# FoundationVision/OmniTokenizer

Measured on AMD Instinct MI355X. Metric: patches/sec encode+decode, higher is better.
Workload: dtype f32 (fp32 operands as 2 fp16 planes, 3 fp16-MFMA products, fp32 accumulate; spatial attention likewise; VQ: fp16-MFMA screen + exact fp32 re-evaluation, ids bit-exact); 1 GPU; C3: B=32/GPU 17x256x256 clips, stage-2 (imagenet_k600 arch: ttww/tttt, pt=4, rope, n_codes=8192), encode + decode; 32 distinct clips per rank; global_batch=32, parallelism=clip-sharded x1

## Files before the change

### omnitokenizer_amd/csrc/common.cpp

```cpp
#include "common.h"
#include "../../include/omnitok_debug.h"
#include <limits.h>
#include <string.h>

namespace omnitok {
static thread_local char g_err[1024] = "";

void set_error(const char *fmt, ...) {
    va_list ap;
    va_start(ap, fmt);
    vsnprintf(g_err, sizeof(g_err), fmt, ap);
    va_end(ap);
}
}

#include <map>
#include <mutex>
#include <utility>

namespace omnitok {
static std::mutex g_attr_mu;
static std::map<std::pair<const void *, int>, int> g_attr_bytes;
static std::map<int, int> g_dev_cus;

int set_max_dynamic_lds(const void *kernel, int bytes) {
    int dev = 0;
    OT_HIP(hipGetDevice(&dev));
    std::lock_guard<std::mutex> lk(g_attr_mu);
    int &have = g_attr_bytes[std::make_pair(kernel, dev)];
    if (bytes > have) {
        OT_HIP(hipFuncSetAttribute(kernel, hipFuncAttributeMaxDynamicSharedMemorySize, bytes));
        have = bytes;
    }
    return OMNITOK_OK;
}

int current_device_cus(int *n_cu) {
    int dev = 0;
    OT_HIP(hipGetDevice(&dev));
    std::lock_guard<std::mutex> lk(g_attr_mu);
    auto it = g_dev_cus.find(dev);
    if (it == g_dev_cus.end()) {
        int n = 0;
        OT_HIP(hipDeviceGetAttribute(&n, hipDeviceAttributeMultiprocessorCount, dev));
        it = g_dev_cus.emplace(dev, n).first;
    }
    *n_cu = it->second;
    return OMNITOK_OK;
}
}

#define OT_OPTIONS(X)                   \
    X(gemm_variant, false, INT_MIN)     \
    X(gemm_lds_pad_kb, false, INT_MIN)  \
    X(gemm_gn, false, INT_MIN)          \
    X(gemm_small, false, INT_MIN)       \
    X(vq_split, false, INT_MIN)         \
    X(vq_variant, false, INT_MIN)       \
    X(vq_screen, false, INT_MIN)        \
    X(vq_screen_split, false, INT_MIN)  \
    X(x3_tile, false, INT_MIN)          \
    X(h2_tile, false, INT_MIN)          \
    X(peg_variant, false, INT_MIN)      \
    X(gemm_mode, true, INT_MIN)         \
    X(attn_mode, true, INT_MIN)         \
    X(attn_h2_variant, false, INT_MIN)  \
    X(attn_vpack, false, INT_MIN)       \
    X(attn_window_mode, false, INT_MIN) \
    X(gemm_pl, true, INT_MIN)           \
    X(qkv_pl, false, INT_MIN)           \
    X(pl_min_tokens, true, INT_MIN)     \
    X(pl_cfg, true, INT_MIN)            \
    X(pl_tail, true, INT_MIN)           \
    X(pl_stagger, false, INT_MIN)       \
    X(sp_small_blocks, true, INT_MIN)   \
    X(temporal_chunk, true, INT_MIN)    \
    X(temporal_fused, false, INT_MIN)   \
    X(temporal_kernel, false, INT_MIN)  \
    X(prevq_fuse, true, INT_MIN)        \
    X(lm_wide_u, true, INT_MIN)         \
    X(lm_balance, true, INT_MIN)        \
    X(lm_ksliced, true, INT_MIN)        \
    X(lm_mfma, true, INT_MIN)           \
    X(lm_mfma_mult, true, INT_MIN)      \
    X(lm_ks_deep, true, INT_MIN)        \
    X(lm_attn_short, true, INT_MIN)     \
    X(lm_attn_waves, true, INT_MIN)     \
    X(lm_loss_chunk_rows, true, 1)

namespace omnitok {
extern long long *g_gemm_trace;
void lm_trace_reset();
#define OT_OPTION_DECL(name, readable, min) extern int g_##name;
OT_OPTIONS(OT_OPTION_DECL)
#undef OT_OPTION_DECL

struct Option {
    const char *name;
    int *value;
    bool readable;
    int min;
};
#define OT_OPTION_ROW(name, readable, min) {#name, &g_##name, readable, min},
static const Option g_options[] = {OT_OPTIONS(OT_OPTION_ROW)};
#undef OT_OPTION_ROW

static const Option *find_option(const char *name) {
    for (const Option &o : g_options)
        if (!strcmp(name, o.name)) return &o;
    return nullptr;
}
}

extern "C" int omnitok_set_option(const char *name, int value) {
    if (!name) return OMNITOK_ERR_INVALID;
    const omnitok::Option *o = omnitok::find_option(name);
    if (!o) {
        omnitok::set_error("set_option: unknown option %s", name);
        return OMNITOK_ERR_INVALID;
    }
    OT_CHECK_ARG(value >= o->min, "set_option: %s %d, expected at least %d", name, value, o->min);
    *o->value = value;
    return OMNITOK_OK;
}

extern "C" int omnitok_get_option(const char *name, int *value) {
    if (!name || !value) return OMNITOK_ERR_INVALID;
    const omnitok::Option *o = omnitok::find_option(name);
    if (!o || !o->readable) {
// ... 16 lines not shown
```

### omnitokenizer_amd/csrc/engine.h

```cpp
#pragma once
#include "common.h"

#include <map>
#include <string>
#include <vector>
#include <algorithm>
#include <cmath>
#include <cstring>
#include <cstdlib>
#include <iterator>

namespace omnitok {

struct DevTensor {
    void *p = nullptr;
    std::vector<int64_t> shape;
    bool is_int64 = false;
    int64_t numel() const {
        int64_t n = 1;
        for (auto s : shape) n *= s;
        return n;
    }
};

// ... 20 lines not shown
    const float *ng, *nb, *wqkv, *wproj, *bproj, *bias_dense;
    const float *wqkv_fold = nullptr, *fold_b = nullptr, *fold_u = nullptr;
    float ln_bound = 0.0f, ao_bound = 0.0f;
    float q_bound = 0.0f, k_bound = 0.0f;
};
struct LayerFF {
    const float *lw, *lb, *w1p, *w2p;
    float ln_bound = 0.0f, h_bound = 0.0f;
};
struct H2W {
    const void *pl = nullptr;
    const float *sc = nullptr;
};
struct ABound {
    float stat = 0.0f;
    const float *dev = nullptr;
    int64_t rpc = 0;
};
struct Layer {
    char kind;
    LayerT t;
    LayerW w;
    LayerFF ff;
    const float *pool_w = nullptr, *pool_b = nullptr;
};

struct Geo {
    bool defer_t, defer_s;
    int p_enc, pt_enc, p_dec, pt_dec, n_pool;
};
struct TransformerW {
    std::vector<Layer> layers;
    const float *og, *ob;
    float out_bound = 0.0f;
};

struct TimingRec {
    std::string name;
    hipEvent_t a, b;
    double work;
};

}

using namespace omnitok;

struct omnitok_engine {
    omnitok_config cfg;
    std::map<std::string, std::vector<int64_t>> spec;
    std::map<std::string, DevTensor> w;
    std::vector<void *> owned;
    std::vector<void *> retired;
    int opt_gemm_mode = -1, opt_attn_mode = -1, opt_attn_vpack = -1, opt_gemm_pl = -1;
    int opt_pl_min_tokens = -1, opt_temporal_chunk = -1;
    bool finalized = false;
    int inner_pad = 0;
    TransformerW enc_s, enc_t, dec_s, dec_t;
    const float *pe_w[2] = {nullptr, nullptr}, *pe_b[2] = {nullptr, nullptr};
    int pe_k[2] = {0, 0}, pe_ld[2] = {0, 0};
    const float *px_w[2] = {nullptr, nullptr}, *px_b[2] = {nullptr, nullptr};
    float *cb_packed = nullptr, *cb_ee = nullptr, *cb_screen = nullptr, *alibi = nullptr;
    float *dq_table = nullptr;
    std::map<int, std::pair<float *, float *>> rope;
    std::map<std::string, float *> bias_tables;
    Buf X, X2, Y, QKV, AO, HD, Z, ST;
    float *ext_ws = nullptr;
    int64_t ext_ws_bytes = 0;
    std::map<const float *, H2W> h2w;
    std::map<const float *, H2W> plw;
    float pe_bound[2] = {0.0f, 0.0f};
    float *bounds = nullptr;
    int bound_next = 0, bound_clips = 0, bound_cap = 0;
    float *range_scratch = nullptr;
    int *err_flag = nullptr;
    bool timing = false;
    std::vector<TimingRec> recs;
    std::vector<hipEvent_t> pool;
};

namespace omnitok {

constexpr int N_BOUND_LAUNCHES = 64;

extern int g_gemm_mode, g_attn_mode, g_attn_vpack, g_gemm_pl, g_pl_min_tokens, g_temporal_chunk, g_prevq_fuse, g_vq_screen, g_temporal_fused;
extern int g_qkv_pl, g_attn_window_mode;

constexpr int64_t PL_BLOCK_BYTES = 8192;
inline int64_t pl_row_offset(int64_t row0, int K) { return (row0 / 64) * (int64_t)(K / 32) * PL_BLOCK_BYTES; }
inline int64_t pad256(int64_t rows) { return (rows + 255) / 256 * 256; }

Geo geometry(const omnitok_config &c);
bool walk_enc_grid(const char *block, int *gh, int *gw, int64_t *peak);
void add_transformer_spec(omnitok_engine *e, const std::string &prefix, const std::string &block, bool rel);
bool key_unused(const omnitok_engine *e, const std::string &k);
int alloc_f(omnitok_engine *e, float **out, int64_t n);
int ensure(Buf &b, int64_t n);
const char *k_embed(const omnitok_config &c);
const char *k_pre_w(const omnitok_config &c);
const char *k_pre_b(const omnitok_config &c);
const char *k_post_w(const omnitok_config &c);
const char *k_post_b(const omnitok_config &c);
const float *W(omnitok_engine *e, const std::string &k);
int build_transformer(omnitok_engine *e, TransformerW &tw, const std::string &prefix, const std::string &block, bool spatial,
                      hipStream_t stream);
int build_patch_operands(omnitok_engine *e, hipStream_t stream);
int get_rope(omnitok_engine *e, int N, const float **cosp, const float **sinp, hipStream_t stream);
int get_bias_table(omnitok_engine *e, const std::string &prefix, int gh, int gw, const float **out, hipStream_t stream);
int gemm_mode_of(const omnitok_engine *e);
int attn_mode_of(const omnitok_engine *e);
int attn_vpack_of(const omnitok_engine *e);
int gemm_pl_of(const omnitok_engine *e, int64_t tokens);
bool x3_ok(const omnitok_engine *e, int N, int K, int flags);
float *next_bounds(omnitok_engine *e);
struct VPack {
    void *planes; int col0, n_tokens, heads; float bound; const float *bound_dev;
};
struct EgGemm {
    const float *a = nullptr, *w = nullptr, *bias = nullptr, *residual = nullptr;
    int64_t lda = 0, ldw = 0, ldr = 0;
    float *c = nullptr;
    int64_t ldc = 0;
    int64_t M = 0;
    int N = 0, K = 0, flags = 0;
    int64_t rpg = 0, gstride = 0, goff = 0;
    ABound ab;
    const float *ln_stats = nullptr, *ln_g = nullptr, *ln_b = nullptr;
    int ln_cols = 0;
    float ln_bound = 0.0f;
    float *c2 = nullptr;
    int64_t ldc2 = 0;
    int split_col = 0;
    const VPack *vpk = nullptr;
};
int eg_gemm(omnitok_engine *e, const EgGemm &g, hipStream_t stream, bool *vpacked = nullptr);
struct PreVqFuse {
    const float *w, *b;
    float *z;
// ... 45 lines not shown
```

### omnitokenizer_amd/csrc/engine.hip

```cpp
#include "engine.h"

namespace omnitok {

int reset_bounds(omnitok_engine *e, int B, hipStream_t stream) {
    if (B > e->bound_cap) {
        if (e->bounds) e->retired.push_back(e->bounds);
        e->bounds = nullptr;
        const int cap = B > 1024 ? B : 1024;
        OT_HIP(hipMalloc(reinterpret_cast<void **>(&e->bounds), (size_t)2 * cap * N_BOUND_LAUNCHES * sizeof(float)));
        e->bound_cap = cap;
    }
    e->bound_clips = B;
    e->bound_next = 0;
    if (int rc = device_fill_u32(e->bounds, 0u, (int64_t)2 * B * N_BOUND_LAUNCHES, stream)) return rc;
    return OMNITOK_OK;
}

void workspace_widths(const omnitok_engine *e, int64_t (&wd)[8]) {
    const omnitok_config &c = e->cfg;
    const int D = c.dim;
    const Geo g = geometry(c);
    const int kenc = ((c.image_channels * g.p_enc * g.p_enc * g.pt_enc + 31) / 32) * 32;
    const int kdec = c.image_channels * g.p_dec * g.p_dec * g.pt_dec;
    const int kmax = kenc > kdec ? kenc : kdec;
// ... 403 lines not shown
extern "C" int64_t omnitok_engine_workspace_need_encode(omnitok_engine *e, int B, int F, int H, int W_) {
    if (!e) return -1;
    const int64_t L = encode_peak_tokens(e, B, F, H, W_);
    return L < 0 ? -1 : workspace_bytes_for(e, L);
}

extern "C" int64_t omnitok_engine_workspace_need_decode(omnitok_engine *e, int B, int T, int gh, int gw) {
    if (!e || T < 1 || gh < 1 || gw < 1) return -1;
    const Geo g = geometry(e->cfg);
    const int T2 = g.defer_t ? 1 + (T - 1) * 2 : T, up = g.defer_s ? 2 : 1;
    return workspace_bytes_for(e, (int64_t)B * T2 * gh * up * gw * up);
}

extern "C" int omnitok_engine_set_workspace(omnitok_engine *e, void *dev_ptr, int64_t bytes) {
    OT_CHECK_ARG(e, "set_workspace: null engine");
    OT_CHECK_ARG((dev_ptr == nullptr) == (bytes == 0) && bytes >= 0, "set_workspace: pointer / size mismatch");
    OT_CHECK_ARG((reinterpret_cast<uintptr_t>(dev_ptr) & 255) == 0, "set_workspace: the block must be 256-byte aligned");
    Buf *bufs[8] = {&e->X, &e->X2, &e->Y, &e->QKV, &e->AO, &e->HD, &e->Z, &e->ST};
    if (!e->ext_ws)
        for (Buf *b : bufs)
            if (b->p) (void)hipFree(b->p);
    for (Buf *b : bufs) {
        b->p = nullptr;
        b->cap = 0;
    }
    e->ext_ws = static_cast<float *>(dev_ptr);
    e->ext_ws_bytes = bytes;
    return OMNITOK_OK;
}

extern "C" int64_t omnitok_engine_workspace_bytes(omnitok_engine *e) {
    int64_t n = 0;
    for (Buf *b : {&e->X, &e->X2, &e->Y, &e->QKV, &e->AO, &e->HD, &e->Z, &e->ST}) n += b->cap * 4;
    return n;
}

extern "C" int omnitok_engine_set_option(omnitok_engine *e, const char *name, int value) {
    OT_CHECK_ARG(e && name, "engine_set_option: null pointer");
    OT_CHECK_ARG(value >= -1, "engine_set_option: value %d (-1 = follow the process default)", value);
    const std::string n(name);
    if (n == "gemm_mode") {
        OT_CHECK_ARG(value <= 2, "engine_set_option: gemm_mode %d", value);
        e->opt_gemm_mode = value;
    } else if (n == "attn_mode") {
        e->opt_attn_mode = value;
    } else if (n == "attn_vpack") {
        e->opt_attn_vpack = value;
    } else if (n == "gemm_pl") {
        e->opt_gemm_pl = value;
    } else if (n == "pl_min_tokens") {
        e->opt_pl_min_tokens = value;
    } else if (n == "temporal_chunk") {
        e->opt_temporal_chunk = value;
    } else {
        set_error("engine_set_option: %s is not a per-engine option (gemm_mode, attn_mode, attn_vpack, gemm_pl, pl_min_tokens, "
                  "temporal_chunk)", name);
        return OMNITOK_ERR_INVALID;
    }
    return OMNITOK_OK;
}

extern "C" int omnitok_engine_set_timing(omnitok_engine *e, int enabled) {
    OT_CHECK_ARG(e, "set_timing: null engine");
    e->timing = enabled != 0;
    return OMNITOK_OK;
}

extern "C" int omnitok_engine_check_ids(omnitok_engine *e, omnitok_stream_t stream_) {
    hipStream_t stream = static_cast<hipStream_t>(stream_);
    int flag = 0;
    OT_HIP(hipMemcpyAsync(&flag, e->err_flag, sizeof(int), hipMemcpyDeviceToHost, stream));
    OT_HIP(hipStreamSynchronize(stream));
    if (flag) {
        if (int rc = device_fill_u32(e->err_flag, 0u, 1, stream)) return rc;
        set_error("decode: token id out of range [0, %d)", e->cfg.n_codes);
        return OMNITOK_ERR_INVALID;
    }
    return OMNITOK_OK;
}

extern "C" int omnitok_engine_timing_report(omnitok_engine *e, char *buf, int buflen) {
    OT_CHECK_ARG(e && buf && buflen > 0, "timing_report: bad arguments");
    OT_HIP(hipDeviceSynchronize());
    struct Acc { int calls = 0; double ms = 0, work = 0; };
    std::map<std::string, Acc> acc;
    for (auto &r : e->recs) {
        float ms = 0;
        (void)hipEventElapsedTime(&ms, r.a, r.b);
        Acc &a = acc[r.name];
        a.calls++;
        a.ms += ms;
        a.work += r.work;
        e->pool.push_back(r.a);
        e->pool.push_back(r.b);
    }
    e->recs.clear();
    std::string s;
    char line[256];
    for (auto &kv : acc) {
        snprintf(line, sizeof(line), "%s %d %.6f %.6e\n", kv.first.c_str(), kv.second.calls, kv.second.ms,
                 kv.second.work);
        s += line;
    }
    strncpy(buf, s.c_str(), buflen - 1);
    buf[buflen - 1] = 0;
    return OMNITOK_OK;
}
```

### omnitokenizer_amd/csrc/engine_run.hip

```cpp
#include "engine.h"

namespace omnitok {

int g_gemm_mode = 2;
int g_attn_mode = 1;
int g_attn_vpack = 1;
int g_gemm_pl = 1;
int g_pl_min_tokens = 0;
int g_temporal_chunk = 0;
int g_prevq_fuse = 1;
int g_temporal_fused = 1;
int g_qkv_pl = 1;
int g_attn_window_mode = 1;

int gemm_mode_of(const omnitok_engine *e) { return e->opt_gemm_mode >= 0 ? e->opt_gemm_mode : g_gemm_mode; }
int attn_mode_of(const omnitok_engine *e) { return e->opt_attn_mode >= 0 ? e->opt_attn_mode : g_attn_mode; }
int attn_vpack_of(const omnitok_engine *e) { return e->opt_attn_vpack >= 0 ? e->opt_attn_vpack : g_attn_vpack; }
int gemm_pl_of(const omnitok_engine *e, int64_t tokens) {
    const int min_tokens = e->opt_pl_min_tokens >= 0 ? e->opt_pl_min_tokens : g_pl_min_tokens;
    return (e->opt_gemm_pl >= 0 ? e->opt_gemm_pl : g_gemm_pl) && tokens >= min_tokens;
}
static int temporal_chunk_of(const omnitok_engine *e) { return e->opt_temporal_chunk >= 0 ? e->opt_temporal_chunk : g_temporal_chunk; }

bool x3_ok(const omnitok_engine *e, int N, int K, int flags) {
    return gemm_mode_of(e) >= 1 && N % 32 == 0 && K % 32 == 0 && !(flags & OMNITOK_GEMM_LEAKY) &&
           (!(flags & OMNITOK_GEMM_GEGLU) || N % 64 == 0);
}

float *next_bounds(omnitok_engine *e) {
    if (e->bound_next >= N_BOUND_LAUNCHES) return nullptr;
    return e->bounds + (int64_t)2 * e->bound_clips * (e->bound_next++);
}

int eg_gemm(omnitok_engine *e, const EgGemm &g, hipStream_t stream, bool *vpacked) {
    omnitok_row_gemm d = {};
    d.a = g.a; d.lda = g.lda; d.w = g.w; d.ldw = g.ldw;
    d.bias = g.bias; d.residual = g.residual; d.ldr = g.ldr; d.c = g.c; d.ldc = g.ldc;
    d.M = g.M; d.N = g.N; d.K = g.K; d.flags = g.flags;
    d.a_rows_per_group = g.rpg; d.a_group_stride = g.gstride; d.a_group_offset = g.goff;
    d.a_bound = g.ab.stat; d.a_bound_dev = g.ab.dev; d.a_bound_stride = 2; d.a_rows_per_clip = g.ab.rpc;
    d.ln_stats = g.ln_stats; d.ln_gamma = g.ln_g; d.ln_beta = g.ln_b; d.ln_cols = g.ln_cols; d.ln_bound = g.ln_bound;
    d.c2 = g.c2; d.ldc2 = g.ldc2; d.split_col = g.split_col;
    if (gemm_mode_of(e) == 2 && g.ab.stat > 0.0f && x3_ok(e, g.N, g.K, g.flags) && (!g.ln_stats || g.ln_bound > 0.0f) &&
        (!g.ab.dev || (g.ab.rpc > 0 && g.ab.rpc % 64 == 0 && g.rpg == 0))) {
        auto it = e->h2w.find(g.w);
        if (it != e->h2w.end() && g.ldw == g.K) {
            d.w = nullptr; d.ldw = 0; d.w_planes = it->second.pl; d.w_scale = it->second.sc;
            if (g.vpk && g.ab.dev && g.ab.rpc % 128 == 0) {
                *vpacked = true;
                d.v_planes = g.vpk->planes; d.v_col0 = g.vpk->col0; d.n_tokens = g.vpk->n_tokens; d.heads = g.vpk->heads;
                d.v_bound = g.vpk->bound; d.v_bound_dev = g.vpk->bound_dev; d.v_bound_stride = 2;
            }
            return omnitok_gemm_h2(&d, stream);
        }
    }
    if (x3_ok(e, g.N, g.K, g.flags)) return omnitok_gemm_x3(&d, stream);
    if (g.ln_stats) {
        set_error("eg_gemm: fused LayerNorm needs the x3 / h2 kernel");
        return OMNITOK_ERR_STATE;
    }
    return omnitok_gemm(&d, stream);
}

static int eg_gemm_pl(omnitok_engine *e, omnitok_pl_gemm g, const float *w, hipStream_t stream) {
    auto it = e->plw.find(w);
    if (it == e->plw.end()) {
        set_error("eg_gemm_pl: weight was not packed for the plane GEMM");
        return OMNITOK_ERR_STATE;
    }
    g.w = it->second.pl;
    g.w_scale = it->second.sc;
    return omnitok_gemm_pl(&g, stream);
}

static H2W pl_cols(const H2W &w, int col0, int K) {
    return H2W{static_cast<const char *>(w.pl) + pl_row_offset(col0, K), w.sc + col0};
}

namespace {

struct AttnPlanes {
    unsigned char *qp, *kp, *vp;
};

struct TBlock {
    float *bs;
    int64_t rpc;
    ABound ab_x, ab_ao;
    float *Q, *KV;
    float qb, kb;
    bool attn_h2;
    AttnPlanes p;
};

struct QkvState {
    bool vpacked = false;
    bool qk_packed = false;
    bool ao_planes = false;
    bool temporal_done = false;
};

struct Run {
    omnitok_engine *e;
    const TransformerW &tw;
    hipStream_t stream;
    const omnitok_config &c;
    const int D, heads, B, T;
    const bool spatial;
    int gh = 0, gw = 0, S = 0;
    int64_t L = 0;
    double gemm_f = 0.0;
    bool fused = false;
    bool pl = false;
    bool ln_planes_ready = false;

    Run(omnitok_engine *e_, const TransformerW &tw_, hipStream_t stream_, int B_, int T_, bool spatial_)
        : e(e_), tw(tw_), stream(stream_), c(e_->cfg), D(e_->cfg.dim), heads(e_->cfg.heads), B(B_), T(T_), spatial(spatial_) {}

    void set_grid(int gh_, int gw_) {
        gh = gh_;
        gw = gw_;
        S = gh * gw;
        L = (int64_t)B * T * S;
        gemm_f = 2.0 * (double)L * D;
    }
    AttnPlanes attn_planes() const {
        unsigned char *kp = reinterpret_cast<unsigned char *>(e->HD.p);
        return AttnPlanes{reinterpret_cast<unsigned char *>(e->Y.p), kp, kp + (size_t)L * D * 4};
    }
    omnitok_pl_gemm qkv_pl_base(const H2W &w) const {
        omnitok_pl_gemm g{};
        g.a = e->X2.p;
        g.a_scale = e->Z.p;
        g.w = w.pl;
        g.w_scale = w.sc;
        g.fold_stats = e->ST.p;
        g.M = L;
        g.K = D;
        return g;
    }

    void decide_flow();
    int pack_rows(const float *src, void *planes, float *scales);
    int gemm_out_pl(const Layer &ly, const void *a_planes, const float *a_scale, float a_const, const float *w, const float *bias);
    int pool_block(const Layer &ly);
    int up_block(const Layer &ly);
    int temporal_block(const Layer &ly);
    int temporal_single_token(const Layer &ly, const TBlock &t);
    int temporal_fused5(const Layer &ly, const TBlock &t);
    int produce_qkv(const Layer &ly, const TBlock &t, QkvState &st);
    int produce_qkv_chunked(const Layer &ly, const TBlock &t, const omnitok_pl_gemm &g, int chunk, QkvState &st);
    int run_attention(const Layer &ly, const TBlock &t, QkvState &st);
    int window_block(const Layer &ly);
    int feed_forward(const Layer &ly);
    int norm_out(bool transpose_out, bool out_planes, const PreVqFuse *pv);
};

void Run::decide_flow() {
    fused = x3_ok(e, 3 * D, D, 0) && D <= 512;
    bool pl_ok = gemm_pl_of(e, L) && gemm_mode_of(e) == 2 && fused && D == 512 && x3_ok(e, 2 * e->inner_pad, D, OMNITOK_GEMM_GEGLU);
    for (const Layer &ly : tw.layers)
        if (!(ly.ff.ln_bound > 0.0f && ly.ff.ln_bound < 1e30f && ly.ff.h_bound > 0.0f && ly.ff.h_bound < 1e30f)) pl_ok = false;
    pl = pl_ok;
}

int Run::pack_rows(const float *src, void *planes, float *scales) {
    OT_RUN("pack_rows", 2.0 * L * D * 4.0, omnitok_pl_pack_rows(src, D, L, D, pad256(L), planes, scales, 0.0f, stream));
    return OMNITOK_OK;
}

int Run::gemm_out_pl(const Layer &ly, const void *a_planes, const float *a_scale, float a_const, const float *w,
                     const float *bias) {
    omnitok_pl_gemm g{};
    g.a = a_planes;
    g.a_scale = a_scale;
    g.a_scale_const = a_const;
    g.bias = bias;
    g.residual = e->X.p;
    g.ldr = D;
    g.c = e->X.p;
    g.ldc = D;
    g.out_planes = e->Y.p;
    g.out_planes_k = D;
    g.out_bound = ly.ff.ln_bound;
    g.ln_gamma = ly.ff.lw;
    g.ln_beta = ly.ff.lb;
    g.ln_eps = 1e-5f;
    g.epilogue = 2;
    g.M = L;
    g.N = D;
    g.K = D;
    OT_RUN("gemm_out", gemm_f * D, eg_gemm_pl(e, g, w, stream));
    ln_planes_ready = true;
    return OMNITOK_OK;
}

int Run::pool_block(const Layer &ly) {
    if (!spatial || gh % 2 || gw % 2) {
        set_error("pooling block '%c' on a %dx%d grid", ly.kind, gh, gw);
        return OMNITOK_ERR_INVALID;
    }
    if (ly.kind == 'l') {
        EgGemm g;
        g.a = e->X.p; g.lda = 4 * D;
        g.w = ly.pool_w; g.ldw = 4 * D;
        g.bias = ly.pool_b;
        g.c = e->X2.p; g.ldc = D;
        g.M = L / 4; g.N = D; g.K = 4 * D;
        g.flags = OMNITOK_GEMM_BIAS;
        OT_RUN("pool", 2.0 * (double)L * D * D, eg_gemm(e, g, stream));
    } else {
        OT_RUN("pool", 1.25 * L * D * 4.0,
               omnitok_token_resample(e->X.p, e->X2.p, ly.kind == 'a' ? 0 : 1, (int64_t)B * T, 1, gh, gw, D, stream));
    }
    std::swap(e->X, e->X2);
    set_grid(gh / 2, gw / 2);
    return OMNITOK_OK;
}

int Run::up_block(const Layer &ly) {
    if (!spatial) {
        set_error("Up block '%c' in a temporal transformer", ly.kind);
        return OMNITOK_ERR_INVALID;
    }
    const float *src = e->X.p;
    if (ly.kind == 'r') {
        EgGemm g;
        g.a = e->X.p; g.lda = D;
        g.w = ly.pool_w; g.ldw = D;
        g.bias = ly.pool_b;
        g.c = e->Y.p; g.ldc = D;
        g.M = L; g.N = D; g.K = D;
        g.flags = OMNITOK_GEMM_BIAS;
        OT_RUN("pool", 2.0 * (double)L * D * D, eg_gemm(e, g, stream));
        src = e->Y.p;
    }
    OT_RUN("pool", 1.25 * 4.0 * L * D * 4.0, omnitok_token_resample(src, e->X2.p, 2, (int64_t)B * T, 1, gh, gw, D, stream));
    std::swap(e->X, e->X2);
    set_grid(gh * 2, gw * 2);
    return OMNITOK_OK;
}

int Run::temporal_block(const Layer &ly) {
    OT_RUN("peg3d", 2.0 * L * D * 4.0,
           omnitok_peg3d(e->X.p, ly.t.peg_w27, ly.t.peg_b, e->X2.p, B, T, gh, gw, D, c.causal_peg, stream));
    std::swap(e->X, e->X2);
    TBlock t;
    t.bs = fused ? next_bounds(e) : nullptr;
    if (fused && !t.bs) {
        set_error("run_transformer: out of range slots");
        return OMNITOK_ERR_STATE;
    }
    t.rpc = L / B;
    t.ab_x = t.bs ? ABound{1.01f, t.bs, t.rpc} : ABound();
    t.ab_ao = t.bs ? ABound{1.01f * ly.t.vnorm, t.bs + 1, t.rpc} : ABound();
    if (!spatial && T == 1) return temporal_single_token(ly, t);
    if (!spatial && T == 5 && pl && g_qkv_pl && g_temporal_fused && t.bs && c.causal_temporal && ly.t.wqk_t &&
        e->plw.count(ly.t.wqk_t) && ly.t.wqkv_fold && e->plw.count(ly.t.wqkv_fold) && S % 64 == 0 && heads * 64 == D &&
        ly.t.vnorm > 0.0f)
        return temporal_fused5(ly, t);
    t.Q = e->QKV.p;
    t.KV = e->QKV.p + L * D;
    t.qb = 1.01f * 8.0f * ly.t.q_amax;
    t.kb = 1.01f * ly.t.k_amax;
    t.attn_h2 = spatial && attn_mode_of(e) == 1 && t.bs && S % 64 == 0 && t.qb > 0.0f && t.kb > 0.0f && ly.t.vnorm > 0.0f &&
                t.qb < 1e30f && t.kb < 1e30f;
    t.p = attn_planes();
    QkvState st;
    if (int rc = produce_qkv(ly, t, st)) return rc;
    if (int rc = run_attention(ly, t, st)) return rc;
    if (pl) {
        const void *ap = e->AO.p;
        if (!st.ao_planes) {
            if (int rc = pack_rows(e->AO.p, e->QKV.p, e->ST.p)) return rc;
            ap = e->QKV.p;
        }
        return gemm_out_pl(ly, ap, e->ST.p, 1.0f, ly.t.wo, nullptr);
    }
    EgGemm g;
    g.a = e->AO.p; g.lda = D;
    g.w = ly.t.wo; g.ldw = D;
    g.residual = e->X.p; g.ldr = D;
    g.c = e->X.p; g.ldc = D;
    g.M = L; g.N = D; g.K = D;
    g.flags = OMNITOK_GEMM_RESIDUAL;
    g.ab = t.ab_ao;
    OT_RUN("gemm_out", gemm_f * D, eg_gemm(e, g, stream));
    return OMNITOK_OK;
}

int Run::temporal_single_token(const Layer &ly, const TBlock &t) {
    if (pl && ly.t.wvo && e->plw.count(ly.t.wvo)) {
        OT_RUN("stats_pack", 2.0 * L * D * 4.0,
               omnitok_stats_pack(e->X.p, L, D, 1e-5f, 0, e->X2.p, pad256(L), e->Z.p, nullptr, nullptr, 0, stream));
        return gemm_out_pl(ly, e->X2.p, e->Z.p, 1.0f, ly.t.wvo, nullptr);
    }
    if (t.bs && gemm_mode_of(e) == 2)
        OT_RUN("row_stats", L * D * 4.0, omnitok_row_stats(e->X.p, L, D, 1e-5f, e->ST.p, t.bs, t.rpc, stream));
    EgGemm v;
    v.a = e->X.p; v.lda = D;
    v.w = ly.t.wkv + (int64_t)D * D; v.ldw = D;
    v.c = e->AO.p; v.ldc = D;
    v.M = L; v.N = D; v.K = D;
    v.ab = t.ab_x;
    OT_RUN("gemm_qkv", gemm_f * D, eg_gemm(e, v, stream));
    if (pl) {
        if (int rc = pack_rows(e->AO.p, e->QKV.p, e->ST.p)) return rc;
        return gemm_out_pl(ly, e->QKV.p, e->ST.p, 1.0f, ly.t.wo, nullptr);
    }
    EgGemm g;
    g.a = e->AO.p; g.lda = D;
    g.w = ly.t.wo; g.ldw = D;
    g.residual = e->X.p; g.ldr = D;
    g.c = e->X.p; g.ldc = D;
    g.M = L; g.N = D; g.K = D;
    g.flags = OMNITOK_GEMM_RESIDUAL;
    g.ab = t.ab_ao;
    OT_RUN("gemm_out", gemm_f * D, eg_gemm(e, g, stream));
    return OMNITOK_OK;
}

int Run::temporal_fused5(const Layer &ly, const TBlock &t) {
    const int64_t nseq = (int64_t)B * S;
    float *P = e->QKV.p, *out_scale = e->QKV.p + nseq * heads * 40;
    OT_RUN("stats_pack", 2.0 * L * D * 4.0,
           omnitok_stats_pack_temporal(e->X.p, nseq, D, 1e-5f, e->X2.p, e->Z.p, e->ST.p, t.bs, S, stream));
    const float *alibi = c.legacy_attention ? e->alibi : nullptr;
    omnitok_pl_gemm g = qkv_pl_base(H2W{});
    g.tp = P;
    g.t_nseq = (int)nseq;
    g.t_heads = heads;
    g.t_alibi = alibi;
    omnitok_pl_gemm q = g;
    const H2W &wqk = e->plw[ly.t.wqk_t];
    q.w = wqk.pl;
    q.w_scale = wqk.sc;
    q.fold_b = ly.t.qk_t_fb;
    q.fold_u = ly.t.qk_t_fu;
    q.N = 2 * D;
    q.epilogue = 6;
    q.q_scale = ly.t.q_scale;
    q.k_scale = ly.t.k_scale;
    q.q_mul = 8.0f;
    OT_RUN("gemm_qkv", gemm_f * 2 * D, omnitok_gemm_pl(&q, stream));
    const H2W wv = pl_cols(e->plw[ly.t.wqkv_fold], 2 * D, D);
    omnitok_pl_gemm v = g;
    v.w = wv.pl;
    v.w_scale = wv.sc;
    v.fold_u = ly.t.fold_u + 2 * D;
    v.N = D;
    v.epilogue = 7;
    v.out_planes = e->AO.p;
    v.out_planes_k = D;
    v.t_out_scale = out_scale;
    v.v_bound = t.ab_ao.stat;
    v.v_bound_dev = t.ab_ao.dev;
    v.v_bound_stride = 2;
    v.t_seqs_per_clip = S;
    OT_RUN("gemm_qkv", gemm_f * D, omnitok_gemm_pl(&v, stream));
    return gemm_out_pl(ly, e->AO.p, out_scale, 1.0f, ly.t.wo, nullptr);
}

int Run::produce_qkv(const Layer &ly, const TBlock &t, QkvState &st) {
    const VPack vpk{t.p.vp, 2 * D, S, heads, t.ab_ao.stat, t.ab_ao.dev};
    const bool qkv_pl = pl && g_qkv_pl && ly.t.wqkv_fold && e->plw.count(ly.t.wqkv_fold) && t.bs;
    if (qkv_pl) {
        OT_RUN("stats_pack", 2.0 * L * D * 4.0,
               omnitok_stats_pack(e->X.p, L, D, 1e-5f, 1, e->X2.p, pad256(L), e->Z.p, e->ST.p, t.bs, t.rpc, stream));
        const H2W &wf = e->plw[ly.t.wqkv_fold];
        omnitok_pl_gemm g = qkv_pl_base(wf);
        g.fold_b = ly.t.fold_b;
        g.fold_u = ly.t.fold_u;
        g.fold_cols = D;
        if (t.attn_h2 && t.rpc % 256 == 0) {
            const float *cosp = nullptr, *sinp = nullptr;
            if (c.spatial_rope)
                if (int rc = get_rope(e, S, &cosp, &sinp, stream)) return rc;
            omnitok_pl_gemm q = g;
            q.N = 2 * D;
            q.epilogue = 4;
            q.qp = t.p.qp;
            q.kp = t.p.kp;
            q.qk_k0 = D;
            q.n_tokens = S;
            q.heads = heads;
            q.rope_cos = cosp;
            q.rope_sin = sinp;
            q.q_scale = ly.t.q_scale;
            q.k_scale = ly.t.k_scale;
            q.q_mul = 8.0f;
            q.q_bound = t.qb;
            q.k_bound = t.kb;
            OT_RUN("gemm_qkv", gemm_f * 2 * D, omnitok_gemm_pl(&q, stream));
            const H2W wv = pl_cols(wf, 2 * D, D);
            omnitok_pl_gemm v = g;
            v.fold_cols = 0;
            v.fold_b = nullptr;
            v.fold_u = ly.t.fold_u + 2 * D;
            v.w = wv.pl;
            v.w_scale = wv.sc;
            v.N = D;
            v.epilogue = 3;
            v.vp = t.p.vp;
            v.n_tokens = S;
            v.heads = heads;
            v.v_bound = t.ab_ao.stat;
            v.v_bound_dev = t.ab_ao.dev;
            v.v_bound_stride = 2;
            v.rows_per_clip = t.rpc;
            OT_RUN("gemm_qkv", gemm_f * D, omnitok_gemm_pl(&v, stream));
            st.vpacked = true;
            st.qk_packed = true;
            return OMNITOK_OK;
        }
        g.N = 3 * D;
        g.epilogue = 0;
        g.c = t.Q;
        g.ldc = D;
        g.c2 = t.KV;
        g.ldc2 = 2 * D;
        g.c_split_n = D;
// ... 310 lines not shown
```

### omnitokenizer_amd/csrc/vq.hip

```cpp
#include "common.h"
#include "h2_common.h"

namespace omnitok {

constexpr int VQ_ROWS_PER_WAVE = 64;
constexpr int VQ_ROWS_PER_BLOCK = 256;
int g_vq_split = 0;
int g_vq_variant = 1;
int g_vq_screen = 1;
int g_vq_screen_split = 0;

__global__ void vq_prepare_kernel(const float *__restrict__ E, int n_codes, float *__restrict__ packed,
                                  float *__restrict__ ee) {
    const int idx = blockIdx.x * blockDim.x + threadIdx.x;
    if (idx >= n_codes * 2) return;
    const int tile = idx >> 6, lane = idx & 63, r32 = lane & 31, hi = lane >> 5;
    const int c = tile * 32 + r32;
    f32x4 a;
#pragma unroll
    for (int s = 0; s < 4; ++s) a[s] = E[c * 8 + 2 * s + hi];
    reinterpret_cast<f32x4 *>(packed)[idx] = a;
    if (hi == 0) {
        float acc = 0.0f;
#pragma unroll
// ... 436 lines not shown
    const int64_t row = ((int64_t)blockIdx.x * blockDim.x + threadIdx.x) >> 4;
    if (row >= n) return;
    float acc[8];
#pragma unroll
    for (int c = 0; c < 8; ++c) acc[c] = 0.0f;
    const float *xr = x + row * D;
    for (int i = l16 * 4; i < D; i += 64) {
        const f32x4 xv = *reinterpret_cast<const f32x4 *>(xr + i);
#pragma unroll
        for (int c = 0; c < 8; ++c) {
            const f32x4 wv = *reinterpret_cast<const f32x4 *>(w + c * D + i);
            acc[c] += prevq_dot4(xv[0], xv[1], xv[2], xv[3], wv[0], wv[1], wv[2], wv[3]);
        }
    }
#pragma unroll
    for (int c = 0; c < 8; ++c) acc[c] = row16_allsum(acc[c]) + b[c];
    if (l2) prevq_l2norm8(acc);
    if (l16 == 0) *reinterpret_cast<f32x4 *>(z + row * 8) = f32x4{acc[0], acc[1], acc[2], acc[3]};
    if (l16 == 1) *reinterpret_cast<f32x4 *>(z + row * 8 + 4) = f32x4{acc[4], acc[5], acc[6], acc[7]};
}

__global__ __launch_bounds__(256) void dequant_post_vq_kernel(const int64_t *__restrict__ ids,
                                                              const float *__restrict__ E, int n_codes,
                                                              const float *__restrict__ w,
                                                              const float *__restrict__ b, float *__restrict__ tok,
                                                              int64_t n, int D, int *err_flag) {
    const int d4n = D >> 2;
    const int64_t gid = (int64_t)blockIdx.x * blockDim.x + threadIdx.x;
    if (gid >= n * d4n) return;
    const int64_t row = gid / d4n;
    const int c4 = (int)(gid % d4n);
    int64_t id = ids[row];
    if (id < 0 || id >= n_codes) {
        if (err_flag) atomicOr(err_flag, 1);
        id = 0;
    }
    const f32x4 e0 = *reinterpret_cast<const f32x4 *>(E + id * 8);
    const f32x4 e1 = *reinterpret_cast<const f32x4 *>(E + id * 8 + 4);
    f32x4 o = reinterpret_cast<const f32x4 *>(b)[c4];
#pragma unroll
    for (int j = 0; j < 4; ++j) {
        const f32x4 w0 = *reinterpret_cast<const f32x4 *>(w + (c4 * 4 + j) * 8);
        const f32x4 w1 = *reinterpret_cast<const f32x4 *>(w + (c4 * 4 + j) * 8 + 4);
        float s = 0.0f;
#pragma unroll
        for (int k = 0; k < 4; ++k) s = fmaf(e0[k], w0[k], s);
#pragma unroll
        for (int k = 0; k < 4; ++k) s = fmaf(e1[k], w1[k], s);
        o[j] += s;
    }
    reinterpret_cast<f32x4 *>(tok)[gid] = o;
}

__global__ __launch_bounds__(256) void gather_rows_kernel(const int64_t *__restrict__ ids,
                                                          const f32x4 *__restrict__ table, int n_codes,
                                                          f32x4 *__restrict__ tok, int64_t n, int d4n, int *err_flag,
                                                          int tr_a, int tr_c) {
    const int64_t gid = (int64_t)blockIdx.x * blockDim.x + threadIdx.x;
    if (gid >= n * d4n) return;
    const int64_t row = gid / d4n;
    const int c4 = (int)(gid % d4n);
    int64_t id = ids[row];
    if (id < 0 || id >= n_codes) {
        if (err_flag) atomicOr(err_flag, 1);
        id = 0;
    }
    int64_t orow = row;
    if (tr_a > 0) {
        const int64_t c = row % tr_c, ba = row / tr_c;
        orow = ((ba / tr_a) * tr_c + c) * tr_a + ba % tr_a;
    }
    __builtin_nontemporal_store(table[id * d4n + c4], tok + orow * d4n + c4);
}

__global__ void iota_i64_kernel(int64_t *__restrict__ out, int n) {
    const int i = blockIdx.x * blockDim.x + threadIdx.x;
    if (i < n) out[i] = i;
}

__global__ __launch_bounds__(256) void vq_embed_st_kernel(const int64_t *__restrict__ ids,
                                                          const float *__restrict__ z, const float *__restrict__ E,
                                                          int64_t B, int64_t thw, float *__restrict__ emb) {
    const int64_t gid = (int64_t)blockIdx.x * blockDim.x + threadIdx.x;
    if (gid >= B * thw) return;
    const int64_t b = gid / thw, s = gid % thw;
    const int64_t id = ids[gid];
#pragma unroll
    for (int c = 0; c < 8; ++c) {
        const float zv = z[gid * 8 + c];
        emb[(b * 8 + c) * thw + s] = __fadd_rn(__fsub_rn(E[id * 8 + c], zv), zv);
    }
}

__global__ __launch_bounds__(256) void vae_sample_kernel(const float *__restrict__ x, const float *__restrict__ w,
                                                         const float *__restrict__ b,
                                                         const float *__restrict__ noise, float *__restrict__ z,
                                                         float *__restrict__ moments, int64_t n, int64_t thw,
                                                         int D) {
    const int l16 = threadIdx.x & 15;
    const int64_t row = ((int64_t)blockIdx.x * blockDim.x + threadIdx.x) >> 4;
    if (row >= n) return;
    float acc[16];
#pragma unroll
    for (int c = 0; c < 16; ++c) acc[c] = 0.0f;
    const float *xr = x + row * D;
    for (int i = l16 * 4; i < D; i += 64) {
        const f32x4 xv = *reinterpret_cast<const f32x4 *>(xr + i);
#pragma unroll
        for (int c = 0; c < 16; ++c) {
            const f32x4 wv = *reinterpret_cast<const f32x4 *>(w + c * D + i);
            acc[c] += (xv[0] * wv[0] + xv[1] * wv[1]) + (xv[2] * wv[2] + xv[3] * wv[3]);
        }
    }
    float mine = 0.0f, other = 0.0f;
#pragma unroll
    for (int c = 0; c < 16; ++c) {
        const float v = row16_allsum(acc[c]) + b[c];
        if (c == l16) mine = v;
        if (c == (l16 ^ 8)) other = v;
    }
    const int64_t bi = row / thw, s = row % thw;
    if (moments) moments[(bi * 16 + l16) * thw + s] = mine;
    if (l16 < 8) {
        float out = mine;
        if (noise) {
// ... 232 lines not shown
    hipLaunchKernelGGL(vq_finalize_kernel, dim3((unsigned)((n + 255) / 256)), dim3(256), 0, stream, ids, n);
    OT_LAUNCH_CHECK("vq_finalize");
    return OMNITOK_OK;
}

extern "C" int omnitok_vq_argmax_cos(const float *z, const float *packed, int64_t n, int n_codes, int64_t *ids,
                                     omnitok_stream_t stream_) {
    hipStream_t stream = static_cast<hipStream_t>(stream_);
    if (n == 0) return OMNITOK_OK;
    OT_CHECK_ARG(z && packed && ids, "vq_argmax_cos: null pointer");
    OT_CHECK_ARG(n_codes % 32 == 0 && n_codes > 0 && n_codes <= 32768, "vq_argmax_cos: n_codes=%d unsupported", n_codes);
    OT_CHECK_ARG(aligned16(z) && aligned16(packed), "vq_argmax_cos: unaligned");
    return launch_vq<VQ_COS>(z, packed, nullptr, n, n_codes, ids, stream);
}

extern "C" int omnitok_vq_argmin_cdist(const float *z, const float *packed, const float *ee, int64_t n, int n_codes,
                                       int64_t *ids, omnitok_stream_t stream_) {
    hipStream_t stream = static_cast<hipStream_t>(stream_);
    if (n == 0) return OMNITOK_OK;
    OT_CHECK_ARG(z && packed && ee && ids, "vq_argmin_cdist: null pointer");
    OT_CHECK_ARG(n_codes % 32 == 0 && n_codes > 0 && n_codes <= 32768, "vq_argmin_cdist: n_codes=%d unsupported",
                 n_codes);
    OT_CHECK_ARG(aligned16(z) && aligned16(packed) && aligned16(ee), "vq_argmin_cdist: unaligned");
    return launch_vq<VQ_EUCLID>(z, packed, ee, n, n_codes, ids, stream);
}

extern "C" int omnitok_dequant_table(const float *codebook, int n_codes, int cdim, const float *w, const float *b,
                                     float *table, int D, int64_t *scratch_ids, omnitok_stream_t stream_) {
    hipStream_t stream = static_cast<hipStream_t>(stream_);
    OT_CHECK_ARG(codebook && w && b && table && scratch_ids, "dequant_table: null pointer");
    OT_CHECK_ARG(cdim == 8 && D % 4 == 0 && n_codes > 0, "dequant_table: need cdim == 8, D %% 4 == 0, n_codes > 0");
    hipLaunchKernelGGL(iota_i64_kernel, dim3((n_codes + 255) / 256), dim3(256), 0, stream, scratch_ids, n_codes);
    OT_LAUNCH_CHECK("iota");
    const int64_t total = (int64_t)n_codes * (D / 4);
    hipLaunchKernelGGL(dequant_post_vq_kernel, dim3((unsigned)((total + 255) / 256)), dim3(256), 0, stream, scratch_ids,
                       codebook, n_codes, w, b, table, (int64_t)n_codes, D, nullptr);
    OT_LAUNCH_CHECK("dequant_table");
    return OMNITOK_OK;
}

extern "C" int omnitok_gather_rows(const int64_t *ids, const float *table, int n_codes, float *tok, int64_t n, int D,
                                   int *err_flag, omnitok_stream_t stream_) {
    return omnitok_gather_rows_transposed(ids, table, n_codes, tok, n, 0, 0, D, err_flag, stream_);
}

extern "C" int omnitok_gather_rows_transposed(const int64_t *ids, const float *table, int n_codes, float *tok, int64_t n,
                                              int a, int c, int D, int *err_flag, omnitok_stream_t stream_) {
    hipStream_t stream = static_cast<hipStream_t>(stream_);
    OT_CHECK_ARG(ids && table && tok, "gather_rows: null pointer");
    OT_CHECK_ARG(D % 4 == 0 && aligned16(table) && aligned16(tok), "gather_rows: need D %% 4 == 0 and 16-byte alignment");
    OT_CHECK_ARG((a == 0 && c == 0) || (a > 0 && c > 0 && n % ((int64_t)a * c) == 0),
                 "gather_rows: %lld rows are not whole [a=%d, c=%d] groups", (long long)n, a, c);
    if (n == 0) return OMNITOK_OK;
    const int64_t total = n * (D / 4);
    hipLaunchKernelGGL(gather_rows_kernel, dim3((unsigned)((total + 255) / 256)), dim3(256), 0, stream, ids,
                       reinterpret_cast<const f32x4 *>(table), n_codes, reinterpret_cast<f32x4 *>(tok), n, D / 4,
                       err_flag, a, c);
    OT_LAUNCH_CHECK("gather_rows");
    return OMNITOK_OK;
}

extern "C" int omnitok_dequant_post_vq(const int64_t *ids, const float *codebook, int n_codes, int cdim,
                                       const float *w, const float *b, float *tok, int64_t n, int D, int *err_flag,
                                       omnitok_stream_t stream_) {
    hipStream_t stream = static_cast<hipStream_t>(stream_);
    OT_CHECK_ARG(ids && codebook && w && b && tok, "dequant_post_vq: null pointer");
    OT_CHECK_ARG(cdim == 8 && D % 4 == 0, "dequant_post_vq: need cdim == 8 and D %% 4 == 0");
    if (n == 0) return OMNITOK_OK;
    const int64_t total = n * (D / 4);
    hipLaunchKernelGGL(dequant_post_vq_kernel, dim3((unsigned)((total + 255) / 256)), dim3(256), 0, stream, ids,
                       codebook, n_codes, w, b, tok, n, D, err_flag);
    OT_LAUNCH_CHECK("dequant_post_vq");
    return OMNITOK_OK;
}

extern "C" int omnitok_vq_embed_st(const int64_t *ids, const float *z, const float *codebook, int cdim, int64_t B,
                                   int64_t thw, float *emb, omnitok_stream_t stream_) {
    hipStream_t stream = static_cast<hipStream_t>(stream_);
    OT_CHECK_ARG(ids && z && codebook && emb && cdim == 8, "vq_embed_st: bad arguments");
    const int64_t total = B * thw;
    if (total == 0) return OMNITOK_OK;
    hipLaunchKernelGGL(vq_embed_st_kernel, dim3((unsigned)((total + 255) / 256)), dim3(256), 0, stream, ids, z,
                       codebook, B, thw, emb);
    OT_LAUNCH_CHECK("vq_embed_st");
    return OMNITOK_OK;
}

extern "C" int omnitok_vae_sample(const float *x, const float *w, const float *b, const float *noise, float *z,
                                  float *moments, int64_t B, int64_t thw, int D, int cdim,
                                  omnitok_stream_t stream_) {
    hipStream_t stream = static_cast<hipStream_t>(stream_);
    const int64_t n = B * thw;
    if (n == 0) return OMNITOK_OK;
    OT_CHECK_ARG(x && w && b && z, "vae_sample: null pointer");
    OT_CHECK_ARG(cdim == 8, "vae_sample: codebook_dim=%d (kernels are built for 8)", cdim);
    OT_CHECK_ARG(D % 64 == 0, "vae_sample: D %% 64 != 0");
    const int64_t threads = n * 16;
    hipLaunchKernelGGL(vae_sample_kernel, dim3((unsigned)((threads + 255) / 256)), dim3(256), 0, stream, x, w, b,
                       noise, z, moments, n, thw, D);
    OT_LAUNCH_CHECK("vae_sample");
    return OMNITOK_OK;
}

extern "C" int omnitok_post_vq(const float *z, int channel_first, int64_t B, int64_t thw, int cdim, const float *w,
                               const float *b, float *tok, int D, omnitok_stream_t stream_) {
    hipStream_t stream = static_cast<hipStream_t>(stream_);
    const int64_t n = B * thw;
    if (n == 0) return OMNITOK_OK;
// ... 12 lines not shown
```

Baseline: 2.758 million patches/s.

## Chunk peg3d with stats_pack per batch slice and row-batch gather kernel

Temporal blocks can now run the peg3d conv and the following stats/pack step interleaved per chunk of clips, so the packed planes are produced while the peg output is still cache-resident. This is controlled by a new peg_chunk option that defaults to 0, so the old full-batch path is used by default. Separately, the gather_rows kernel is rewritten so each wave handles four rows. It loads the ids and computes the destination indices once per row instead of per element, and issues all four row loads before the stores. The chunking adds launches, and the gather change makes the lanes idle when D/4 is less than 64.

```diff
diff --git a/omnitokenizer_amd/csrc/common.cpp b/omnitokenizer_amd/csrc/common.cpp
--- a/omnitokenizer_amd/csrc/common.cpp
+++ b/omnitokenizer_amd/csrc/common.cpp
@@ -75,6 +75,7 @@
     X(pl_stagger, false, INT_MIN)       \
     X(sp_small_blocks, true, INT_MIN)   \
     X(temporal_chunk, true, INT_MIN)    \
+    X(peg_chunk, true, INT_MIN)         \
     X(temporal_fused, false, INT_MIN)   \
     X(temporal_kernel, false, INT_MIN)  \
     X(prevq_fuse, true, INT_MIN)        \
diff --git a/omnitokenizer_amd/csrc/engine.h b/omnitokenizer_amd/csrc/engine.h
--- a/omnitokenizer_amd/csrc/engine.h
+++ b/omnitokenizer_amd/csrc/engine.h
@@ -96,7 +96,7 @@
     std::vector<void *> owned;
     std::vector<void *> retired;
     int opt_gemm_mode = -1, opt_attn_mode = -1, opt_attn_vpack = -1, opt_gemm_pl = -1;
-    int opt_pl_min_tokens = -1, opt_temporal_chunk = -1;
+    int opt_pl_min_tokens = -1, opt_temporal_chunk = -1, opt_peg_chunk = -1;
     bool finalized = false;
     int inner_pad = 0;
     TransformerW enc_s, enc_t, dec_s, dec_t;
@@ -126,7 +126,7 @@
 
 constexpr int N_BOUND_LAUNCHES = 64;
 
-extern int g_gemm_mode, g_attn_mode, g_attn_vpack, g_gemm_pl, g_pl_min_tokens, g_temporal_chunk, g_prevq_fuse, g_vq_screen, g_temporal_fused;
+extern int g_gemm_mode, g_attn_mode, g_attn_vpack, g_gemm_pl, g_pl_min_tokens, g_temporal_chunk, g_peg_chunk, g_prevq_fuse, g_vq_screen, g_temporal_fused;
 extern int g_qkv_pl, g_attn_window_mode;
 
 constexpr int64_t PL_BLOCK_BYTES = 8192;
diff --git a/omnitokenizer_amd/csrc/engine.hip b/omnitokenizer_amd/csrc/engine.hip
--- a/omnitokenizer_amd/csrc/engine.hip
+++ b/omnitokenizer_amd/csrc/engine.hip
@@ -479,9 +479,11 @@
         e->opt_pl_min_tokens = value;
     } else if (n == "temporal_chunk") {
         e->opt_temporal_chunk = value;
+    } else if (n == "peg_chunk") {
+        e->opt_peg_chunk = value;
     } else {
         set_error("engine_set_option: %s is not a per-engine option (gemm_mode, attn_mode, attn_vpack, gemm_pl, pl_min_tokens, "
-                  "temporal_chunk)", name);
+                  "temporal_chunk, peg_chunk)", name);
         return OMNITOK_ERR_INVALID;
     }
     return OMNITOK_OK;
diff --git a/omnitokenizer_amd/csrc/engine_run.hip b/omnitokenizer_amd/csrc/engine_run.hip
--- a/omnitokenizer_amd/csrc/engine_run.hip
+++ b/omnitokenizer_amd/csrc/engine_run.hip
@@ -8,6 +8,7 @@
 int g_gemm_pl = 1;
 int g_pl_min_tokens = 0;
 int g_temporal_chunk = 0;
+int g_peg_chunk = 0;
 int g_prevq_fuse = 1;
 int g_temporal_fused = 1;
 int g_qkv_pl = 1;
@@ -21,6 +22,7 @@
     return (e->opt_gemm_pl >= 0 ? e->opt_gemm_pl : g_gemm_pl) && tokens >= min_tokens;
 }
 static int temporal_chunk_of(const omnitok_engine *e) { return e->opt_temporal_chunk >= 0 ? e->opt_temporal_chunk : g_temporal_chunk; }
+static int peg_chunk_of(const omnitok_engine *e) { return e->opt_peg_chunk >= 0 ? e->opt_peg_chunk : g_peg_chunk; }
 
 bool x3_ok(const omnitok_engine *e, int N, int K, int flags) {
     return gemm_mode_of(e) >= 1 && N % 32 == 0 && K % 32 == 0 && !(flags & OMNITOK_GEMM_LEAKY) &&
@@ -83,7 +85,11 @@
     unsigned char *qp, *kp, *vp;
 };
 
+enum XPack { XP_NONE = 0, XP_SINGLE, XP_FUSED5, XP_QKV };
+
 struct TBlock {
+    XPack pack = XP_NONE;
+    bool packed = false;
     float *bs;
     int64_t rpc;
     ABound ab_x, ab_ao;
@@ -146,6 +152,7 @@
     int pool_block(const Layer &ly);
     int up_block(const Layer &ly);
     int temporal_block(const Layer &ly);
+    int pack_x(const TBlock &t, int c0, int nb);
     int temporal_single_token(const Layer &ly, const TBlock &t);
     int temporal_fused5(const Layer &ly, const TBlock &t);
     int produce_qkv(const Layer &ly, const TBlock &t, QkvState &st);
@@ -241,10 +248,25 @@
     return OMNITOK_OK;
 }
 
+int Run::pack_x(const TBlock &t, int c0, int nb) {
+    const int64_t r0 = (int64_t)c0 * t.rpc, Lc = (int64_t)nb * t.rpc;
+    const int64_t m_pad = (c0 + nb == B ? pad256(L) : r0 + Lc) - r0;
+    const float *x = e->X.p + r0 * D;
+    char *planes = reinterpret_cast<char *>(e->X2.p) + pl_row_offset(r0, D);
+    float *bs = t.bs ? t.bs + 2 * c0 : nullptr;
+    if (t.pack == XP_FUSED5)
+        OT_RUN("stats_pack", 2.0 * Lc * D * 4.0,
+               omnitok_stats_pack_temporal(x, (int64_t)nb * S, D, 1e-5f, planes, e->Z.p + r0, e->ST.p + 2 * r0, bs, S, stream));
+    else if (t.pack == XP_QKV)
+        OT_RUN("stats_pack", 2.0 * Lc * D * 4.0,
+               omnitok_stats_pack(x, Lc, D, 1e-5f, 1, planes, m_pad, e->Z.p + r0, e->ST.p + 2 * r0, bs, t.rpc, stream));
+    else
+        OT_RUN("stats_pack", 2.0 * Lc * D * 4.0,
+               omnitok_stats_pack(x, Lc, D, 1e-5f, 0, planes, m_pad, e->Z.p + r0, nullptr, nullptr, 0, stream));
+    return OMNITOK_OK;
+}
+
 int Run::temporal_block(const Layer &ly) {
-    OT_RUN("peg3d", 2.0 * L * D * 4.0,
-           omnitok_peg3d(e->X.p, ly.t.peg_w27, ly.t.peg_b, e->X2.p, B, T, gh, gw, D, c.causal_peg, stream));
-    std::swap(e->X, e->X2);
     TBlock t;
     t.bs = fused ? next_bounds(e) : nullptr;
     if (fused && !t.bs) {
@@ -254,11 +276,35 @@
     t.rpc = L / B;
     t.ab_x = t.bs ? ABound{1.01f, t.bs, t.rpc} : ABound();
     t.ab_ao = t.bs ? ABound{1.01f * ly.t.vnorm, t.bs + 1, t.rpc} : ABound();
-    if (!spatial && T == 1) return temporal_single_token(ly, t);
-    if (!spatial && T == 5 && pl && g_qkv_pl && g_temporal_fused && t.bs && c.causal_temporal && ly.t.wqk_t &&
-        e->plw.count(ly.t.wqk_t) && ly.t.wqkv_fold && e->plw.count(ly.t.wqkv_fold) && S % 64 == 0 && heads * 64 == D &&
-        ly.t.vnorm > 0.0f)
-        return temporal_fused5(ly, t);
+    const bool single = !spatial && T == 1;
+    const bool fused5 = !spatial && T == 5 && pl && g_qkv_pl && g_temporal_fused && t.bs && c.causal_temporal && ly.t.wqk_t &&
+                        e->plw.count(ly.t.wqk_t) && ly.t.wqkv_fold && e->plw.count(ly.t.wqkv_fold) && S % 64 == 0 &&
+                        heads * 64 == D && ly.t.vnorm > 0.0f;
+    if (single)
+        t.pack = pl && ly.t.wvo && e->plw.count(ly.t.wvo) ? XP_SINGLE : XP_NONE;
+    else if (fused5)
+        t.pack = XP_FUSED5;
+    else
+        t.pack = pl && g_qkv_pl && ly.t.wqkv_fold && e->plw.count(ly.t.wqkv_fold) && t.bs ? XP_QKV : XP_NONE;
+
+    const float *peg_in = e->X.p;
+    float *peg_out = e->X2.p;
+    std::swap(e->X, e->X2);
+    const int chunk = t.pack != XP_NONE ? peg_chunk_of(e) : 0;
+    if (chunk > 0 && chunk < B && t.rpc % 64 == 0) {
+        for (int c0 = 0; c0 < B; c0 += chunk) {
+            const int nb = std::min(chunk, B - c0);
+            const int64_t off = (int64_t)c0 * t.rpc * D;
+            OT_RUN("peg3d", 2.0 * nb * t.rpc * D * 4.0,
+                   omnitok_peg3d(peg_in + off, ly.t.peg_w27, ly.t.peg_b, peg_out + off, nb, T, gh, gw, D, c.causal_peg, stream));
+            if (int rc = pack_x(t, c0, nb)) return rc;
+        }
+        t.packed = true;
+    } else {
+        OT_RUN("peg3d", 2.0 * L * D * 4.0, omnitok_peg3d(peg_in, ly.t.peg_w27, ly.t.peg_b, peg_out, B, T, gh, gw, D, c.causal_peg, stream));
+    }
+    if (single) return temporal_single_token(ly, t);
+    if (fused5) return temporal_fused5(ly, t);
     t.Q = e->QKV.p;
     t.KV = e->QKV.p + L * D;
     t.qb = 1.01f * 8.0f * ly.t.q_amax;
@@ -290,9 +336,9 @@
 }
 
 int Run::temporal_single_token(const Layer &ly, const TBlock &t) {
-    if (pl && ly.t.wvo && e->plw.count(ly.t.wvo)) {
-        OT_RUN("stats_pack", 2.0 * L * D * 4.0,
-               omnitok_stats_pack(e->X.p, L, D, 1e-5f, 0, e->X2.p, pad256(L), e->Z.p, nullptr, nullptr, 0, stream));
+    if (t.pack == XP_SINGLE) {
+        if (!t.packed)
+            if (int rc = pack_x(t, 0, B)) return rc;
         return gemm_out_pl(ly, e->X2.p, e->Z.p, 1.0f, ly.t.wvo, nullptr);
     }
     if (t.bs && gemm_mode_of(e) == 2)
@@ -323,8 +369,8 @@
 int Run::temporal_fused5(const Layer &ly, const TBlock &t) {
     const int64_t nseq = (int64_t)B * S;
     float *P = e->QKV.p, *out_scale = e->QKV.p + nseq * heads * 40;
-    OT_RUN("stats_pack", 2.0 * L * D * 4.0,
-           omnitok_stats_pack_temporal(e->X.p, nseq, D, 1e-5f, e->X2.p, e->Z.p, e->ST.p, t.bs, S, stream));
+    if (!t.packed)
+        if (int rc = pack_x(t, 0, B)) return rc;
     const float *alibi = c.legacy_attention ? e->alibi : nullptr;
     omnitok_pl_gemm g = qkv_pl_base(H2W{});
     g.tp = P;
@@ -363,10 +409,9 @@
 
 int Run::produce_qkv(const Layer &ly, const TBlock &t, QkvState &st) {
     const VPack vpk{t.p.vp, 2 * D, S, heads, t.ab_ao.stat, t.ab_ao.dev};
-    const bool qkv_pl = pl && g_qkv_pl && ly.t.wqkv_fold && e->plw.count(ly.t.wqkv_fold) && t.bs;
-    if (qkv_pl) {
-        OT_RUN("stats_pack", 2.0 * L * D * 4.0,
-               omnitok_stats_pack(e->X.p, L, D, 1e-5f, 1, e->X2.p, pad256(L), e->Z.p, e->ST.p, t.bs, t.rpc, stream));
+    if (t.pack == XP_QKV) {
+        if (!t.packed)
+            if (int rc = pack_x(t, 0, B)) return rc;
         const H2W &wf = e->plw[ly.t.wqkv_fold];
         omnitok_pl_gemm g = qkv_pl_base(wf);
         g.fold_b = ly.t.fold_b;
diff --git a/omnitokenizer_amd/csrc/vq.hip b/omnitokenizer_amd/csrc/vq.hip
--- a/omnitokenizer_amd/csrc/vq.hip
+++ b/omnitokenizer_amd/csrc/vq.hip
@@ -512,25 +512,40 @@
     reinterpret_cast<f32x4 *>(tok)[gid] = o;
 }
 
+constexpr int GR_ROWS = 4;
 __global__ __launch_bounds__(256) void gather_rows_kernel(const int64_t *__restrict__ ids,
                                                           const f32x4 *__restrict__ table, int n_codes,
                                                           f32x4 *__restrict__ tok, int64_t n, int d4n, int *err_flag,
                                                           int tr_a, int tr_c) {
-    const int64_t gid = (int64_t)blockIdx.x * blockDim.x + threadIdx.x;
-    if (gid >= n * d4n) return;
-    const int64_t row = gid / d4n;
-    const int c4 = (int)(gid % d4n);
-    int64_t id = ids[row];
-    if (id < 0 || id >= n_codes) {
-        if (err_flag) atomicOr(err_flag, 1);
-        id = 0;
-    }
-    int64_t orow = row;
-    if (tr_a > 0) {
-        const int64_t c = row % tr_c, ba = row / tr_c;
-        orow = ((ba / tr_a) * tr_c + c) * tr_a + ba % tr_a;
-    }
-    __builtin_nontemporal_store(table[id * d4n + c4], tok + orow * d4n + c4);
+    const int lane = threadIdx.x & 63;
+    const int wave = __builtin_amdgcn_readfirstlane(threadIdx.x >> 6);
+    const int64_t row0 = ((int64_t)blockIdx.x * 4 + wave) * GR_ROWS;
+    const f32x4 *src[GR_ROWS];
+    f32x4 *dst[GR_ROWS];
+#pragma unroll
+    for (int r = 0; r < GR_ROWS; ++r) {
+        const int64_t row = row0 + r < n ? row0 + r : n - 1;
+        int64_t id = ids[row];
+        if (id < 0 || id >= n_codes) {
+            if (err_flag && lane == 0 && row0 + r < n) atomicOr(err_flag, 1);
+            id = 0;
+        }
+        int64_t orow = row;
+        if (tr_a > 0) {
+            const int64_t c = row % tr_c, ba = row / tr_c;
+            orow = ((ba / tr_a) * tr_c + c) * tr_a + ba % tr_a;
+        }
+        src[r] = table + id * d4n;
+        dst[r] = tok + orow * d4n;
+    }
+    for (int c4 = lane; c4 < d4n; c4 += 64) {
+        f32x4 v[GR_ROWS];
+#pragma unroll
+        for (int r = 0; r < GR_ROWS; ++r) v[r] = src[r][c4];
+#pragma unroll
+        for (int r = 0; r < GR_ROWS; ++r)
+            if (row0 + r < n) __builtin_nontemporal_store(v[r], dst[r] + c4);
+    }
 }
 
 __global__ void iota_i64_kernel(int64_t *__restrict__ out, int n) {
@@ -869,8 +884,9 @@
     OT_CHECK_ARG((a == 0 && c == 0) || (a > 0 && c > 0 && n % ((int64_t)a * c) == 0),
                  "gather_rows: %lld rows are not whole [a=%d, c=%d] groups", (long long)n, a, c);
     if (n == 0) return OMNITOK_OK;
-    const int64_t total = n * (D / 4);
-    hipLaunchKernelGGL(gather_rows_kernel, dim3((unsigned)((total + 255) / 256)), dim3(256), 0, stream, ids,
+    const int64_t blocks = (n + 4 * GR_ROWS - 1) / (4 * GR_ROWS);
+    OT_CHECK_ARG(blocks < (1ll << 31), "gather_rows: %lld rows", (long long)n);
+    hipLaunchKernelGGL(gather_rows_kernel, dim3((unsigned)blocks), dim3(256), 0, stream, ids,
                        reinterpret_cast<const f32x4 *>(table), n_codes, reinterpret_cast<f32x4 *>(tok), n, D / 4,
                        err_flag, a, c);
     OT_LAUNCH_CHECK("gather_rows");
```

Result: no change. 2.759 million patches/s (median of 4 runs) (+0.0%).
